# flo-audio/flo

Hardware: AMD Instinct MI355X
Metric: Msamples/s encoded (44.1k stereo, q=high) (higher is better)
Workload: dtype f32

## Files before the change

### diag/lds_model.py

```python
#!/usr/bin/env python3
import argparse
import re
from collections import Counter

import numpy as np

N, HOP, NB = 2048, 1024, 25
SLOT_CAP = 96
ROW = 1024
EDGES = np.array([0, 100, 200, 300, 400, 510, 630, 770, 920, 1080, 1270, 1480, 1720, 2000, 2320, 2700, 3150, 3700,
                  4400, 5300, 6400, 7700, 9500, 12000, 15500, 20500], dtype=np.float32)

R_WIN, R_TW, R_F1, R_F2, R_LANE, R_KEEP, R_DST, R_S10 = 0, 8, 12, 16, 20, 21, 25, 32


def bands(rate):
    res = np.float32(rate) / np.float32(N)
    band = []
    for k in range(HOP):
        f = (np.float32(k) + np.float32(0.5)) * res
        b = NB - 1
        for i in range(1, 26):
            if f < EDGES[i]:
                b = i - 1
# ... 14 lines not shown
                slot_band.append(band[k])
    dirty = 0
    for m in lane_bnd:
        dirty |= m
    band_slot0, s = [], 0
    for b in range(NB):
        band_slot0.append(s)
        while s < len(slot_band) and slot_band[s] == b:
            s += 1
    band_slot0.append(s)
    return lane_bnd, lane_slot0, band_slot0, dirty


G128 = [[0, 1, 2, 3, 12, 13, 14, 15] + list(range(20, 28)), [4, 5, 6, 7, 8, 9, 10, 11, 16, 17, 18, 19] + list(range(28, 32))]
G128 = G128 + [[l + 32 for l in g] for g in G128]
G32 = [list(range(0, 32)), list(range(32, 64))]


def contig(n):
    return [list(range(i, i + n)) for i in range(0, 64, n)]


RULES = {
    "ds_read_b32": [(G32, 1, 32)], "ds_write_b32": [(G32, 1, 32)], "ds_write_b16": [(G32, 1, 32)],
    "ds_read_b64": [(G32, 2, 64)], "ds_read_b128": [(G128, 4, 64)],
    "ds_read2_b32": [(G32, 1, 32), (G32, 1, 32)], "ds_write2_b32": [(G32, 1, 32), (G32, 1, 32)],
    "ds_read2_b64": [(contig(16), 2, 32), (contig(16), 2, 32)],
    "ds_write_b64": [(contig(16), 2, 32)], "ds_write_b128": [(contig(8), 4, 32)],
}


def cost(kind, addrs):
    acc = RULES[kind]
    lists = addrs if len(acc) == 2 else [addrs]
    cyc = base = 0
    for (groups, dw, nbank), ad in zip(acc, lists):
        for g in groups:
            per_bank = {}
            for l in g:
                if ad[l] is None:
                    continue
                for i in range(dw):
                    d = ad[l] // 4 + i
                    per_bank.setdefault(d % nbank, set()).add(d)
            cyc += max([len(v) for v in per_bank.values()] or [1])
            base += 1
    return cyc, cyc - base


def lanes(f):
    return [f(l) for l in range(64)]


def sites(rate, layout):
    lane_bnd, lane_slot0, band_slot0, dirty = band_tables(rate)
    row = lambda r, off=0: lanes(lambda l: r * ROW + 16 * l + off)
    uni = lambda a: lanes(lambda l: a)
    one = lambda a: [a] + [None] * 63
    S = []
    S += [("frame", "peek consumed / coef counters", "ds_read_b32", uni(0x8000))] * 2
    S += [("frame", "kRowS10 (uniform)", "ds_read_b128", uni(R_S10 * ROW))] * 2
    if layout == "old":
        S += [("frame", "rcount: kRowLane .z", "ds_read_b32", row(R_LANE, 8))]
    else:
        S += [("frame", "rcount: kRowS10 dword 64 + lane", "ds_read_b32", lanes(lambda l: R_S10 * ROW + 256 + 4 * l))]
    for ph, rr in (("fft pass 1", R_F1), ("fft pass 2", R_F2)):
        S += [(ph, "twiddle rows", "ds_read_b128", row(rr + k)) for k in range(3)]
        S += [(ph, "twiddle row 4 (.xy)", "ds_read_b64", row(rr + 3))]
    X = 0x10000
    for ka in range(8):
        S += [("fft exchange 1", "writes", "ds_write_b128", lanes(lambda l: X + 16 * ((8 * ka + (l & 7)) * 9 + (l >> 3))))]
    for r in range(8):
        S += [("fft exchange 1", "reads", "ds_read_b128", lanes(lambda l: X + 16 * (l * 9 + r)))]
    T = X + 16000
    S += [("masking pass", "ts_ready peek", "ds_read_b32", uni(0x8004))]
    S += [("masking pass", "ts (tl, sf)", "ds_write2_b32", [lanes(lambda l: T + 16 * (l & 31) + 4 * (l >> 5) + o if (l & 31) < 25 else None) for o in (0, 8)])]
    S += [("masking pass", "sfwh", "ds_write_b16", lanes(lambda l: T + 1024 + 2 * l if (l & 31) < 25 else None))]
    S += [("masking pass", "alive", "ds_write_b64", one(T + 1200))]
    S += [("masking pass", "ts_ready", "ds_write_b32", one(0x8004))]
    for kb in range(8):
        S += [("fft exchange 2", "writes", "ds_write_b128", lanes(lambda l: X + 16 * (((l >> 3) + 8 * kb) * 9 + (l & 7))))]
    for r in range(8):
        S += [("fft exchange 2", "reads", "ds_read_b128", lanes(lambda l: X + 16 * (l * 9 + r)))]
    pl = lambda l: 2 * l + 2 * (l >> 3)
    for r in range(8):
        if layout == "old" or r % 2 == 0:
            if layout == "old":
                S += [("post-rotation", "twiddle rows (half rows)", "ds_read_b64", row(R_TW + r // 2, 8 * (r & 1)))]
            else:
                S += [("post-rotation", "twiddle rows", "ds_read_b128", row(R_TW + r // 2))]
        S += [("post-rotation", "transpose writes (2m)", "ds_write_b64", lanes(lambda l: X + 8 * (pl(l) + 144 * r)))]
        S += [("post-rotation", "transpose writes (1023-2m)", "ds_write_b64", lanes(lambda l: X + 8 * (1149 - pl(l) - 144 * r)))]
    for q in range(8):
        S += [("post-rotation", "transpose reads", "ds_read_b128", lanes(lambda l: X + 16 * (9 * l) + 16 * q))]
    S += [("band statistics", "coef_ready", "ds_write_b32", one(0x8008))]
    es = [e for e in range(16) if (dirty >> e) & 1]
    if layout == "old":
        for rr in (R_KEEP, R_DST):
            for g in range(4):
                comp = [e - 4 * g for e in es if 4 * g <= e < 4 * g + 4 and (rr == R_DST or e < 15)]
                i = 0
                while i < len(comp):
                    if i + 1 < len(comp) and comp[i + 1] == comp[i] + 1 and comp[i] % 2 == 1:
                        S += [("band statistics", "keep / dst rows (dword pieces)", "ds_read2_b32", [row(rr + g, 4 * comp[i]), row(rr + g, 4 * comp[i] + 4)])]
                        i += 2
                    elif i + 1 < len(comp) and comp[i + 1] == comp[i] + 1:
                        S += [("band statistics", "keep / dst rows (dword pieces)", "ds_read_b64", row(rr + g, 4 * comp[i]))]
                        i += 2
                    else:
                        S += [("band statistics", "keep / dst rows (dword pieces)", "ds_read_b32", row(rr + g, 4 * comp[i]))]
                        i += 1
    else:
        S += [("band statistics", "keep / dst rows (whole rows)", "ds_read_b128", row(rr + g)) for rr in (R_KEEP, R_DST) for g in range(4)]
    SL = X + 9216
    for e in es:
        def dst(l, e=e):
            m = lane_bnd[l]
            if (m >> e) & 1:
                return SL + 16 * (lane_slot0[l] + bin(m & ((1 << e) - 1)).count("1"))
            return SL + 16 * (SLOT_CAP + l)
        S += [("band statistics", "slot stores", "ds_write_b128", lanes(dst))]
    zero = SLOT_CAP + 64
    for u in range(12):
        def src(l, u=u):
            b = min(l & 31, 24)
            bs0 = band_slot0[b] + (l >> 5)
            bs1 = band_slot0[b + 1] if (l & 31) < 25 else 0
            s = bs0 + 2 * u
            return SL + 16 * (s if s < bs1 else zero)
        S += [("band statistics", "slot gathers", "ds_read_b128", lanes(src))]
    for r in range(8):
        S += [("fold", "window rows", "ds_read_b128", row(R_WIN + r))]
    if layout == "old":
        for k in range(4):
            S += [("fold", "twiddle rows (read2_b64)", "ds_read2_b64", [row(R_TW + k), row(R_TW + k, 8)])]
    else:
        S += [("fold", "twiddle rows", "ds_read_b128", row(R_TW + k)) for k in range(4)]
    return S


def isa_mix(path):
    txt = open(path).read().split("\n")
    start = next(i for i, t in enumerate(txt) if re.match(r"^_ZN3flo20lossy_chain2q_kernelILb0ELj(\d+)ELb0EE.*:", t)
                 and "Lj65535E" not in t)
    body = txt[start:]
    e = next(i for i, t in enumerate(body) if re.match(r"^\.LBB\d+_\d+:.*_clEjS\d_S\d_S\d_S\d_\.exit", t))
    a = max(i for i, t in enumerate(body[:e]) if re.match(r"^\.LBB\d+_\d+:\s+; %\.lr\.ph\d*$", t))
    lab = body[e].split(":")[0]
    c = next(i for i, t in enumerate(body) if i > a and re.search(r"s_cbranch\w*\s+" + re.escape(lab) + r"\b", t))
    b = next(i for i, t in enumerate(body) if i > e and re.match(r"^\.LBB", t))
    mix, cold = Counter(), Counter()
    for i in range(a, b):
        m = re.search(r"\b(ds_[a-z0-9_]+)", body[i])
        if m:
            (cold if c <= i < e else mix)[m.group(1)] += 1
    return mix, cold


def main():
    ap = argparse.ArgumentParser()
    ap.add_argument("--rate", type=int, default=44100)
    ap.add_argument("--layout", default="old", choices=["old", "new"])
    ap.add_argument("--isa")
    a = ap.parse_args()
    S = sites(a.rate, a.layout)
    tab = {}
    tot_c = tot_x = 0
    for ph, site, kind, ad in S:
        c, x = cost(kind, ad)
        k = (ph, site, kind)
        n, cc, xx = tab.get(k, (0, 0, 0))
        tab[k] = (n + 1, cc + c, xx + x)
        tot_c += c
        tot_x += x
    print(f"{'phase':16} {'site':38} {'instruction':14} {'n':>3} {'array':>6} {'conflict':>8}")
    for (ph, site, kind), (n, c, x) in tab.items():
        print(f"{ph:16} {site:38} {kind:14} {n:3d} {c:6d} {x:8d}")
    print(f"{'transform wave, one stereo frame':70} {len(S):3d} {tot_c:6d} {tot_x:8d}")
    if a.isa:
        mix, cold = isa_mix(a.isa)
        model = Counter(kind for _, _, kind, _ in S)
        print("ISA mix (one frame):", dict(sorted(mix.items())), " cold loop (not run at this rate):", dict(cold))
        print("model mix          :", dict(sorted(model.items())))


if __name__ == "__main__":
    main()
```

### flo_amd/csrc/lossy_device.hpp

```cpp
#pragma once
#include <hip/hip_runtime.h>
#include <stdint.h>

#include "pack_rows.h"

namespace flo {


struct LossyDevTables {
    const float4 *pack;
    const float4 *pack_g;
    const float4 *pack_ext;
    const float *ath_db;
    const uint8_t *band;
    const float *band_count;
    const float *s10d;
    const uint32_t *lane_bnd;
    const uint32_t *lane_slot0;
    const uint32_t *band_slot0;
    int max_band_slots;
    uint32_t dirty;
    float smr_thr;
    int q_transparent;
};

constexpr int kXchStride = 9;
constexpr int kXchFloats = 64 * kXchStride * 2;
#ifdef FLO_COEF_PAD16
constexpr int kCoefFloats = 1280;
#else
constexpr int kCoefFloats = 1152;
#endif
constexpr int kSlotCap = 96;
constexpr int kFrameCap = 4352;

template <int CH>
struct WaveLds {
    union {
        float xch[CH][kXchFloats];
        float coef[CH][kCoefFloats];
        int16_t qbuf[CH][1024];
    } u;
    float2 slots[CH][kSlotCap + 64 + 1];
    float2 bandv[CH][32];
    float band_s[CH][32];
};

__device__ __forceinline__ float4 pack_row(const float4 *p) {
    typedef float v4f __attribute__((ext_vector_type(4)));
    v4f v = *reinterpret_cast<const v4f *>(p);
    asm("" : "+v"(v));
    return make_float4(v.x, v.y, v.z, v.w);
}

__device__ __forceinline__ int lane_id() { return (int)(threadIdx.x & 63); }
__device__ __forceinline__ int lane_id_opaque() {
// ... 315 lines not shown
#pragma unroll
        for (int ch = 0; ch < CH; ch++) {
            float R = fmaf(-zi[ch][r], w.y, -(zr[ch][r] * w.x));
            float I = fmaf(zi[ch][r], w.x, -(zr[ch][r] * w.y));
            coef[ch][p0] = R;
            coef[ch][p1] = I;
        }
    }
    wave_sync();
#pragma unroll
    for (int ch = 0; ch < CH; ch++) {
#ifdef FLO_COEF_PAD16
        const float4 *p = reinterpret_cast<const float4 *>(&coef[ch][20 * lane]);
#else
        const float4 *p = reinterpret_cast<const float4 *>(&coef[ch][16 * lane + 4 * (lane >> 1)]);
#endif
#pragma unroll
        for (int q = 0; q < 4; q++) {
            float4 v = p[q];
            c[ch][4 * q + 0] = v.x;
            c[ch][4 * q + 1] = v.y;
            c[ch][4 * q + 2] = v.z;
            c[ch][4 * q + 3] = v.w;
        }
    }
    wave_sync();
}

typedef float v2f __attribute__((ext_vector_type(2)));
__device__ __forceinline__ v2f fma2(v2f a, v2f b, v2f c) { return __builtin_elementwise_fma(a, b, c); }
__device__ __forceinline__ v2f fma2_na_hi_nc(v2f a, v2f w, v2f c) {
    v2f r;
    asm("v_pk_fma_f32 %0, %1, %2, %3 op_sel:[0,1,0] op_sel_hi:[1,1,1] neg_lo:[1,0,1] neg_hi:[1,0,1]" : "=v"(r) : "v"(a), "v"(w), "v"(c));
    return r;
}
__device__ __forceinline__ v2f fma2_a_hi_c(v2f a, v2f w, v2f c) {
    v2f r;
    asm("v_pk_fma_f32 %0, %1, %2, %3 op_sel:[0,1,0] op_sel_hi:[1,1,1]" : "=v"(r) : "v"(a), "v"(w), "v"(c));
    return r;
}
__device__ __forceinline__ v2f mul2_hi(v2f a, v2f w) {
    v2f r;
    asm("v_pk_mul_f32 %0, %1, %2 op_sel:[0,1] op_sel_hi:[1,1]" : "=v"(r) : "v"(a), "v"(w));
    return r;
}
__device__ __forceinline__ v2f fma2_a_hi_nc(v2f a, v2f w, v2f c) {
    v2f r;
    asm("v_pk_fma_f32 %0, %1, %2, %3 op_sel:[0,1,0] op_sel_hi:[1,1,1] neg_lo:[0,0,1] neg_hi:[0,0,1]" : "=v"(r) : "v"(a), "v"(w), "v"(c));
    return r;
}
__device__ __forceinline__ v2f splat2(float x) { return (v2f){x, x}; }

constexpr int kXch4 = 64 * kXchStride;
constexpr int kCoef2 = 1024 + 2 * 64;

__device__ __forceinline__ void dft8_2(v2f *xr, v2f *xi) {
    const v2f s = splat2(0.70710678118654752440f);
    v2f a0r = xr[0] + xr[4], a0i = xi[0] + xi[4];
    v2f a1r = xr[0] - xr[4], a1i = xi[0] - xi[4];
    v2f a2r = xr[2] + xr[6], a2i = xi[2] + xi[6];
    v2f a3r = xr[2] - xr[6], a3i = xi[2] - xi[6];
    v2f a4r = xr[1] + xr[5], a4i = xi[1] + xi[5];
    v2f a5r = xr[1] - xr[5], a5i = xi[1] - xi[5];
    v2f a6r = xr[3] + xr[7], a6i = xi[3] + xi[7];
    v2f a7r = xr[3] - xr[7], a7i = xi[3] - xi[7];
    v2f b0r = a0r + a2r, b0i = a0i + a2i;
    v2f b2r = a0r - a2r, b2i = a0i - a2i;
    v2f b1r = a1r + a3i, b1i = a1i - a3r;
    v2f b3r = a1r - a3i, b3i = a1i + a3r;
    v2f c0r = a4r + a6r, c0i = a4i + a6i;
    v2f c2r = a4r - a6r, c2i = a4i - a6i;
    v2f c1r = a5r + a7i, c1i = a5i - a7r;
    v2f c3r = a5r - a7i, c3i = a5i + a7r;
    const v2f e1r = c1r + c1i, e1i = c1i - c1r;
    const v2f e3r = c3i - c3r, e3i = c3r + c3i;
    xr[0] = b0r + c0r; xi[0] = b0i + c0i;
    xr[4] = b0r - c0r; xi[4] = b0i - c0i;
    xr[1] = fma2(e1r, s, b1r); xi[1] = fma2(e1i, s, b1i);
    xr[5] = fma2(-e1r, s, b1r); xi[5] = fma2(-e1i, s, b1i);
    xr[2] = b2r + c2i; xi[2] = b2i - c2r;
    xr[6] = b2r - c2i; xi[6] = b2i + c2r;
    xr[3] = fma2(e3r, s, b3r); xi[3] = fma2(-e3i, s, b3i);
    xr[7] = fma2(-e3r, s, b3r); xi[7] = fma2(e3i, s, b3i);
}

__device__ __forceinline__ void cmul_2(v2f &xr, v2f &xi, float wr, float wi) {
    const v2f WR = splat2(wr), WI = splat2(wi);
    v2f r = fma2(xr, WR, -(xi * WI));
    v2f i = fma2(xr, WI, xi * WR);
    xr = r;
    xi = i;
}
__device__ __forceinline__ void cmul_2_pair(v2f &xr, v2f &xi, v2f w) {
    const v2f WR = splat2(w.x);
    v2f r = fma2(xr, WR, -mul2_hi(xi, w));
    v2f i = fma2_a_hi_c(xr, w, xi * WR);
    xr = r;
    xi = i;
}

struct NoShadow { __device__ __forceinline__ void operator()() const {} };
template <typename F = NoShadow>
__device__ __forceinline__ void fft512_2(const int lane, v2f (&zr)[8], v2f (&zi)[8], float4 *x4, const LossyDevTables &T, F &&shadow = F()) {
    dft8_2(zr, zi);
#pragma unroll
    for (int kk = 0; kk < 4; kk++) {
        const float4 w = T.pack[(kRowF1 + kk) * 64 + lane];
// ... 35 lines not shown
        wave_sync();
    }
    dft8_2(zr, zi);
}

__device__ __forceinline__ void load_half_fast_2(const int lane, const float *__restrict__ pcm, long long s0, v2f (&he)[8], v2f (&ho)[8]) {
    const char *base0 = reinterpret_cast<const char *>(pcm + s0 * 2);
    const char *base1 = base0 + 4096;
    const unsigned va = 16u * (unsigned)lane, vb = 16u * (unsigned)(63 - lane);
#pragma unroll
    for (int r = 0; r < 8; r++) {
        const int rr = r & 3;
        const char *pe = (r < 4 ? base1 : base0) + va + 1024 * rr;
        const char *po = (r < 4 ? base0 : base1) + vb + (3080 - 1024 * rr);
        const float2 a = *reinterpret_cast<const float2 *>(pe);
        const float2 b = *reinterpret_cast<const float2 *>(po);
        he[r] = (v2f){a.x, a.y};
        ho[r] = (v2f){b.x, b.y};
    }
}

__device__ __forceinline__ void fold_2(const int lane, const v2f (&ae)[8], const v2f (&ao)[8], const v2f (&be)[8], const v2f (&bo)[8],
                                       v2f (&zr)[8], v2f (&zi)[8], const LossyDevTables &T) {
    float4 t4;
#pragma unroll
    for (int r = 0; r < 8; r++) {
        const float4 ww = T.pack[(kRowWin + r) * 64 + lane];
        const v2f wae = splat2(ww.x), wao = splat2(ww.y), wbe = splat2(ww.z);
        const v2f whi = {ww.z, ww.w};
        if (!(r & 1)) t4 = pack_row(&T.pack[(kRowTw + (r >> 1)) * 64 + lane]);
        const v2f wx = splat2((r & 1) ? t4.z : t4.x);
        const v2f thi = {t4.z, t4.w};
        v2f re, im;
        if (r < 4) {
            re = fma2_na_hi_nc(bo[r], whi, be[r] * wbe);
            im = fma2(ao[r], wao, -(ae[r] * wae));
        } else {
            re = fma2(-ao[r], wao, ae[r] * wae);
            im = fma2_na_hi_nc(bo[r], whi, be[r] * wbe);
        }
        if (r & 1) {
            zr[r] = fma2_na_hi_nc(im, thi, re * wx);
            zi[r] = fma2_a_hi_nc(re, thi, im * wx);
        } else {
            const v2f wy = splat2(t4.y);
            zr[r] = fma2(-im, wy, -(re * wx));
            zi[r] = fma2(re, wy, -(im * wx));
        }
    }
}

__device__ __forceinline__ void post_rotate_transpose_2(const int lane, const v2f (&zr)[8], const v2f (&zi)[8], float2 *c2,
                                                        v2f (&c)[16], const LossyDevTables &T) {
    const int pl = 2 * lane + 2 * (lane >> 3);
    float2 *const w0 = c2 + pl;
    float2 *const w1 = c2 + (1149 - 7 * 144) - pl;
    float4 t4;
#pragma unroll
    for (int r = 0; r < 8; r++) {
        if (!(r & 1)) t4 = pack_row(&T.pack[(kRowTw + (r >> 1)) * 64 + lane]);
        const v2f wx = splat2((r & 1) ? t4.z : t4.x);
        v2f R, I;
        if (r & 1) {
            const v2f thi = {t4.z, t4.w};
            R = fma2_na_hi_nc(zi[r], thi, zr[r] * wx);
            I = fma2(zi[r], wx, -mul2_hi(zr[r], thi));
        } else {
            const v2f wy = splat2(t4.y);
            R = fma2(-zi[r], wy, -(zr[r] * wx));
            I = fma2(zi[r], wx, -(zr[r] * wy));
        }
        w0[144 * r] = make_float2(R.x, R.y);
        w1[144 * (7 - r)] = make_float2(I.x, I.y);
    }
    wave_sync();
    const float4 *p = reinterpret_cast<const float4 *>(&c2[18 * lane]);
#pragma unroll
    for (int q = 0; q < 8; q++) {
        const float4 v = p[q];
        c[2 * q] = (v2f){v.x, v.y};
        c[2 * q + 1] = (v2f){v.z, v.w};
    }
    wave_sync();
}

struct LaneConst {
    float rcount;
};

__device__ __forceinline__ void load_lane_const(const int lane, LaneConst &L, const LossyDevTables &T) {
    L.rcount = T.pack[kRowLane * 64 + lane].z;
}

constexpr int kZeroSlot = kSlotCap + 64;

template <int CH>
__device__ __forceinline__ void band_stats(const int lane, const float (&c)[CH][16], float2 (*slots)[kSlotCap + 64 + 1],
                                           const LossyDevTables &T, float (&energy)[CH], float (&bmax)[CH]) {
    float kp[16];
    uint32_t dv[16], so[12];
#pragma unroll
    for (int g = 0; g < 4; g++) {
        const float4 keep = T.pack[(kRowKeep + g) * 64 + lane];
        const float4 dsto = T.pack[(kRowDst + g) * 64 + lane];
        kp[4 * g + 0] = keep.x, kp[4 * g + 1] = keep.y, kp[4 * g + 2] = keep.z, kp[4 * g + 3] = keep.w;
        dv[4 * g + 0] = __float_as_uint(dsto.x), dv[4 * g + 1] = __float_as_uint(dsto.y);
        dv[4 * g + 2] = __float_as_uint(dsto.z), dv[4 * g + 3] = __float_as_uint(dsto.w);
    }
#pragma unroll
    for (int g = 0; g < 3; g++) {
        const float4 lst = T.pack[(kRowLst + g) * 64 + lane];
        so[4 * g + 0] = __float_as_uint(lst.x), so[4 * g + 1] = __float_as_uint(lst.y);
        so[4 * g + 2] = __float_as_uint(lst.z), so[4 * g + 3] = __float_as_uint(lst.w);
    }
    __builtin_amdgcn_sched_barrier(0);
    float acc[CH], mx[CH];
#pragma unroll
    for (int ch = 0; ch < CH; ch++) {
        acc[ch] = 0.f;
        mx[ch] = 0.f;
    }
#pragma unroll
    for (int e = 0; e < 16; e++) {
#pragma unroll
        for (int ch = 0; ch < CH; ch++) {
            acc[ch] = fmaf(c[ch][e], c[ch][e], acc[ch]);
            mx[ch] = max_abs_raw(mx[ch], c[ch][e]);
            *reinterpret_cast<float2 *>(reinterpret_cast<char *>(slots[ch]) + dv[e]) = make_float2(acc[ch], mx[ch]);
            acc[ch] *= kp[e];
            mx[ch] *= kp[e];
        }
    }
    wave_sync();
    float2 v[CH][12];
// ... 929 lines not shown
```

### flo_amd/csrc/lossy_kernels.hip

```cpp
#include <assert.h>
#include <stdlib.h>

#include <mutex>
#include <set>
#include <type_traits>
#include <utility>

#include "crc_device.hpp"
#include "lossy_device.hpp"
#include "lossy_kernels.hpp"
#include "../../include/flo_synth.h"

#ifndef FLO_ABLATE
#define FLO_ABLATE 0
#endif
#ifndef FLO_SKIP
#define FLO_SKIP 0
#endif
#ifndef FLO_ABLATE3
#define FLO_ABLATE3 0
#endif
#define FLO_KEEP(x) asm volatile("" ::"v"(x))
#ifdef FLO_STAMPS
#define STAMP(i)                                                                                  \
// ... 419 lines not shown
                unsigned long long beg, len;
                crc_slice_range(total, A.parts, p, beg, len);
                const uint32_t r = crc_slice_reg<64>(tab, skip, blk_pow, byte_pow, data + beg, len, (unsigned)lane, nullptr);
                if (lane == 0) A.part_reg[(unsigned long long)clip * A.parts + p] = r;
            }
            if (lane == 0) A.crc_ready[clip] = A.epoch;
        }
        unsigned long long e = 0;
        if (lane == 0) {
            const unsigned tail = __hip_atomic_load(A.next_clip + 1, __ATOMIC_RELAXED, __HIP_MEMORY_SCOPE_AGENT);
            const unsigned head = __hip_atomic_load(A.next_clip + 2, __ATOMIC_RELAXED, __HIP_MEMORY_SCOPE_AGENT);
            if (head < tail) {
                const unsigned h = __hip_atomic_fetch_add(A.next_clip + 2, 1u, __ATOMIC_RELAXED, __HIP_MEMORY_SCOPE_AGENT);
                if (h < (unsigned)A.n_clips) e = __hip_atomic_load(A.done_q + h, __ATOMIC_RELAXED, __HIP_MEMORY_SCOPE_AGENT);
            }
        }
        const unsigned tag = (unsigned)__builtin_amdgcn_readfirstlane((int)(unsigned)(e >> 32));
        clip = (unsigned)__builtin_amdgcn_readfirstlane((int)(unsigned)e);
        if (tag != A.epoch || clip >= (unsigned)A.n_clips) return;
        __builtin_amdgcn_fence(__ATOMIC_ACQUIRE, "agent");
        asm volatile("s_waitcnt vmcnt(0)" ::: "memory");
        total = __hip_atomic_load(A.clip_bytes + clip, __ATOMIC_RELAXED, __HIP_MEMORY_SCOPE_AGENT);
    }
}

template <bool COEFFS, uint32_t DIRTY, bool DBG>
__global__ __launch_bounds__(FLO_C2X_THREADS) void lossy_chain2q_kernel(LossyArgs A, int clips_per_wg) {
    extern __shared__ __attribute__((aligned(16))) uint8_t lds_raw[];
    const int tid = (int)threadIdx.x;
    const int lane = tid & 63;
    {
        float4 *dstp = reinterpret_cast<float4 *>(lds_raw);
        for (int i = tid; i < kPackRowsHotT * 64; i += (int)blockDim.x) dstp[i] = A.T.pack[i];
        for (int i = tid; i < clips_per_wg; i += (int)blockDim.x) {
            Clip2qLds &c0 = *reinterpret_cast<Clip2qLds *>(lds_raw + kPackBytesHotT + (size_t)i * sizeof(Clip2qLds));
            c0.coef_ready = 0;
            c0.ts_ready = 0;
            c0.consumed = 0;
            c0.clip_seq = 0;
        }
        if (A.clear_next && blockIdx.x == 0 && tid == 0)
            A.clear_next[0] = A.clear_next[1] = A.clear_next[2] = 0;
    }
    __syncthreads();
    const int wv = __builtin_amdgcn_readfirstlane(tid >> 6);
    const int cl = wv % clips_per_wg;
    Clip2qLds &cs = *reinterpret_cast<Clip2qLds *>(lds_raw + kPackBytesHotT + (size_t)cl * sizeof(Clip2qLds));
    uint32_t fbase = 0, seq = 0;
    if (wv >= clips_per_wg) {
#ifndef FLO_PRIO_P
#define FLO_PRIO_P 1
#endif
        __builtin_amdgcn_s_setprio(FLO_PRIO_P);
        typedef __attribute__((address_space(3))) v4f lds_v4f;
        float athn[16];
        uint32_t ts_a[16];
        {
            const uint32_t ts0 = (uint32_t)(uintptr_t)cs.ts[0];
#pragma unroll
            for (int q = 0; q < 4; q++) {
                const float4 a4 = A.T.pack[(kRowAthN + q) * 64 + lane];
                const float4 b4 = A.T.pack[(kRowBoN + q) * 64 + lane];
                athn[4 * q + 0] = a4.x, athn[4 * q + 1] = a4.y, athn[4 * q + 2] = a4.z, athn[4 * q + 3] = a4.w;
                ts_a[4 * q + 0] = ts0 + __float_as_uint(b4.x), ts_a[4 * q + 1] = ts0 + __float_as_uint(b4.y);
                ts_a[4 * q + 2] = ts0 + __float_as_uint(b4.z), ts_a[4 * q + 3] = ts0 + __float_as_uint(b4.w);
            }
        }
        const uint32_t *const blk_g = reinterpret_cast<const uint32_t *>(A.T.pack + kRowBlk * 64);
        const uint32_t cf_a = (uint32_t)(uintptr_t)cs.u.coef2 + 16u * (uint32_t)lane + 16u * ((uint32_t)lane >> 3);
        uint8_t *const stage = cs.stage;
        const uint32_t tab_a = (uint32_t)(uintptr_t)cs.packtab;
        v4f cf[8];
        bool have = false;
        unsigned done_clip = ~0u;
        unsigned long long done_bytes = 0;
        for (;;) {
            unsigned got = 0;
            if (lane == 0) got = atomicAdd(A.next_clip, 1u);
            const unsigned clip = (unsigned)__builtin_amdgcn_readfirstlane((int)got);
            if (lane == 0) cs.clip_cur = clip;
            set_counter(&cs.clip_seq, ++seq);
            if (A.crc_ready) {
                if (clip >= (unsigned)A.n_clips) {
                    tail_crc(A, reinterpret_cast<uint32_t *>(&cs.u), lane, done_clip, done_bytes);
                    return;
                }
                if (done_clip != ~0u) tail_publish(A, done_clip, lane);
            }
            if (clip >= (unsigned)A.n_clips) return;
            const unsigned hops = A.clip_hops[clip];
            const unsigned long long frame0 = A.clip_frame0[clip];
            uint8_t *gout = A.out + A.out_off[clip];
            unsigned long long written = 0;
            uint32_t pend = 0, tailb = 0;
#ifdef FLO_STAMPS
            unsigned long long st_sum[16] = {0, 0, 0, 0, 0, 0, 0, 0, 0, 0, 0, 0, 0, 0, 0, 0}, st_last;
            asm volatile("s_memtime %0\n\ts_waitcnt lgkmcnt(0)" : "=s"(st_last)::"memory");
#endif
            for (unsigned h = 0; h < hops; h++) {
                const int ln = lane_id_opaque();
                const uint32_t g = fbase + h;
                auto take_next = [&]() __attribute__((always_inline)) {
                    if (!have && (uint32_t)__builtin_amdgcn_readfirstlane((int)peek_counter(&cs.coef_ready)) >= g + 2) {
#pragma unroll
                        for (int k = 0; k < 8; k++) cf[k] = *reinterpret_cast<const lds_v4f *>((uintptr_t)(cf_a + 1152u * (uint32_t)k));
                        set_counter(&cs.consumed, g + 2);
                        have = true;
                    }
                };
                uint32_t blk[8];
                {
                    const uint32_t *bp = blk_g;
                    asm volatile("" : "+s"(bp));
#pragma unroll
                    for (int q = 0; q < 8; q++) blk[q] = bp[q];
                }
                if (!have) {
                    wait_counter<FLO_PSLEEP>(&cs.coef_ready, g + 1);
#pragma unroll
                    for (int k = 0; k < 8; k++) cf[k] = *reinterpret_cast<const lds_v4f *>((uintptr_t)(cf_a + 1152u * (uint32_t)k));
                    set_counter(&cs.consumed, g + 1);
                }
                STAMP(0);
#ifdef FLO_STAMPS
                const unsigned long long st_frame0 = st_last;
#endif
                wait_counter<FLO_PSLEEP>(&cs.ts_ready, g + 1);
                STAMP(5);
                const uint32_t par = g & 1u;
                const uint32_t sfw_both = cs.sfwh[par][ln >> 5][ln & 31];
                const uint32_t alive = (uint32_t)__builtin_amdgcn_readfirstlane((int)(cs.alive[par][0] | cs.alive[par][1]));
                uint32_t xd[2][8];
#if (FLO_SKIP & 64) == 0
                if (par) quantise_nat<512>(cf, ts_a, athn, alive, blk, xd);
                else quantise_nat<0>(cf, ts_a, athn, alive, blk, xd);
#else
#pragma unroll
                for (int q = 0; q < 8; q++) { xd[0][q] = __float_as_uint(cf[q].x) & alive & 0x00010001u; xd[1][q] = __float_as_uint(cf[q].y) & blk[q] & 0x00010001u; }
#endif
                have = false;
                take_next();
                STAMP(1);
                if (DBG && A.dbg_q) {
#pragma unroll
                    for (int ch = 0; ch < 2; ch++) {
                        uint32_t *dq = reinterpret_cast<uint32_t *>(A.dbg_q + ((frame0 + h) * 2 + ch) * 1024);
#pragma unroll
                        for (int k = 0; k < 8; k++) dq[64 * k + ln] = xd[ch][k];
                    }
                }
                if (ln < (int)pend) stage[ln] = (uint8_t)tailb;
                uint8_t *f = stage + pend;
                const uint32_t f_a = (uint32_t)(uintptr_t)f;
                if ((ln & 31) < 25) {
                    uint8_t *p = f + 12 + 50 * (ln >> 5) + 2 * (ln & 31);
                    lds_st8<0>(p, sfw_both);
                    lds_st8<1>(p, sfw_both >> 8);
                }
                uint32_t tot[2];
                uint32_t pos = 112;
#pragma unroll
                for (int ch = 0; ch < 2; ch++) {
#if (FLO_SKIP & 32) == 0
                    uint32_t t = sparse_item_pack(ln, xd[ch], f_a + pos + 4u, tab_a);
#ifdef FLO_STAMPS
                    if (t == kSparseFallback) st_sum[6] += 1;
#endif
                    if (t == kSparseFallback) t = sparse_block_pack(ln, xd[ch], f_a + pos + 4u, tab_a);
#else
                    uint32_t t = 3u + ((xd[ch][0] | xd[ch][3]) & 1u);
                    FLO_KEEP(xd[ch][1]); FLO_KEEP(xd[ch][2]); FLO_KEEP(xd[ch][4]); FLO_KEEP(xd[ch][5]); FLO_KEEP(xd[ch][6]); FLO_KEEP(xd[ch][7]);
#endif
                    if (t == kSparseFallback) {
// ... 102 lines not shown
        asm volatile("s_memtime %0\n\ts_waitcnt lgkmcnt(0)" : "=s"(st_last)::"memory");
#endif
        v2f zr[8], zi[8];
        if (!COEFFS) fold_2(lane_id_opaque(), ae, ao, be, bo, zr, zi, T);
        float pend_e = 0.f, pend_m = 0.f;
        auto mask_publish = [&](const int ln, const uint32_t gp, const unsigned hp, const float energy1, const float bmax1,
                                const float rcount, const float4 sd0, const float4 sd1) __attribute__((always_inline)) {
            const int bnd = ln & 31, up = ln >> 5;
#if (FLO_SKIP & 16) == 0
            const float bm = bmax1;
            const float sfv1 = bm > 1e-10f ? __fdiv_rn(30000.0f, bm) : 1.0f;
            const uint32_t sfw1 = sf_word(sfv1);
            const float a = spread_threshold_2r(ln, energy1, rcount, sd0, sd1, T);
            const float sl = max_raw(a, prev * 0.7f);
            prev = sl;
            const float tl1 = masking_amplitude(sl, T.smr_thr);
#else
            const float bm = bmax1, tl1 = energy1 * 1e-3f + rcount + sd0.x + sd1.y, sfv1 = bm * 100.f + 1.f;
            const uint32_t sfw1 = __float_as_uint(tl1) >> 16;
#endif
            const unsigned long long al = __ballot(bnd < 25 && bm > tl1);
            if (bnd < 25) {
                typedef __attribute__((address_space(3))) float lds_f32;
                const uint32_t ts_s = (uint32_t)__builtin_amdgcn_readfirstlane((int)(uint32_t)(uintptr_t)cs.ts[gp & 1u]);
                lds_f32 *tp = reinterpret_cast<lds_f32 *>((uintptr_t)(ts_s + 16u * (uint32_t)bnd + 4u * (uint32_t)up));
                tp[0] = tl1;
                tp[2] = sfv1;
                cs.sfwh[gp & 1u][up][bnd] = (uint16_t)sfw1;
            }
            if (ln == 0) {
                cs.alive[gp & 1u][0] = (uint32_t)al;
                cs.alive[gp & 1u][1] = (uint32_t)(al >> 32);
            }
            if (DBG && A.dbg_sfw && bnd < 25) A.dbg_sfw[((frame0 + hp) * 2 + up) * 25 + bnd] = (unsigned short)sfw1;
            set_counter(&cs.ts_ready, gp + 1);
        };
        auto frame_body = [&](const unsigned h, v2f (&ne)[8], v2f (&no)[8], v2f (&fe)[8], v2f (&fo)[8]) __attribute__((always_inline)) {
            const int ln = lane_id_opaque();
            const uint32_t g = fbase + h;
            FLO_MARK("frame_begin");
            const uint32_t consumed_early = peek_counter(&cs.consumed);
            const float4 sd0 = T.pack[kRowS10 * 64], sd1 = T.pack[kRowS10 * 64 + 1];
            const float rcount = reinterpret_cast<const float *>(T.pack + kRowS10 * 64)[64 + ln];
            v2f c[16];
            if (COEFFS) {
#pragma unroll
                for (int q = 0; q < 4; q++) {
                    const float4 v0 = reinterpret_cast<const float4 *>(A.in_coeffs + ((frame0 + h) * 2 + 0) * 1024 + 16 * ln)[q];
                    const float4 v1 = reinterpret_cast<const float4 *>(A.in_coeffs + ((frame0 + h) * 2 + 1) * 1024 + 16 * ln)[q];
                    c[4 * q] = (v2f){v0.x, v1.x}; c[4 * q + 1] = (v2f){v0.y, v1.y};
                    c[4 * q + 2] = (v2f){v0.z, v1.z}; c[4 * q + 3] = (v2f){v0.w, v1.w};
                }
                if ((uint32_t)__builtin_amdgcn_readfirstlane((int)consumed_early) < g) wait_counter(&cs.consumed, g);
                float4 *p = reinterpret_cast<float4 *>(&cs.u.coef2[18 * ln]);
#pragma unroll
                for (int q = 0; q < 8; q++) p[q] = make_float4(c[2 * q].x, c[2 * q].y, c[2 * q + 1].x, c[2 * q + 1].y);
                wave_sync();
            } else {
                load_half_fast_2(ln, pcm, (long long)(h + 1) * 1024, ne, no);
                FLO_MARK("prefetch_done");
                STAMP(1);
                if ((uint32_t)__builtin_amdgcn_readfirstlane((int)consumed_early) < g) wait_counter(&cs.consumed, g);
                STAMP(7);
#if (FLO_SKIP & 8) == 0
                fft512_2(ln, zr, zi, cs.u.xch4, T, [&]() __attribute__((always_inline)) {
                    if (h > 0) mask_publish(ln, g - 1u, h - 1u, pend_e, pend_m, rcount, sd0, sd1);
                });
#else
                if (h > 0) mask_publish(ln, g - 1u, h - 1u, pend_e, pend_m, rcount, sd0, sd1);
#endif
                FLO_MARK("fft_done");
                STAMP(2);
#if (FLO_SKIP & 4) == 0
                post_rotate_transpose_2(ln, zr, zi, cs.u.coef2, c, T);
#else
#pragma unroll
                for (int e = 0; e < 8; e++) { c[2 * e] = zr[e]; c[2 * e + 1] = zi[e]; }
#endif
                FLO_MARK("postrot_done");
                STAMP(3);
                if (DBG && A.dbg_coeffs) {
#pragma unroll
                    for (int ch = 0; ch < 2; ch++) {
                        float *d = A.dbg_coeffs + ((frame0 + h) * 2 + ch) * 1024 + 16 * ln;
#pragma unroll
                        for (int e = 0; e < 16; e++) d[e] = ch ? c[e].y : c[e].x;
                    }
                }
            }
            set_counter(&cs.coef_ready, g + 1);
            float energy1, bmax1;
#if (FLO_SKIP & 1) == 0
            band_stats_2<DIRTY, kSoPre>(ln, c, cs.slot, T, energy1, bmax1, so_pre);
#else
            energy1 = c[0].x + c[5].y;
            bmax1 = c[1].x + c[7].y;
#endif
            FLO_MARK("bandstats_done");
            STAMP(4);
            if (COEFFS) {
                mask_publish(ln, g, h, energy1, bmax1, rcount, sd0, sd1);
            } else {
                pend_e = energy1, pend_m = bmax1;
#if (FLO_SKIP & 128) == 0
                fold_2(ln, fe, fo, ne, no, zr, zi, T);
#else
#pragma unroll
                for (int r = 0; r < 8; r++) { zr[r] = fe[r] + ne[r]; zi[r] = fo[r] - no[r]; }
#endif
// ... 985 lines not shown
```

Before: 674,000.

## Split LDS coefficient buffer into even/odd padded planes to reduce bank conflicts

Replaces the padded interleaved coefficient buffer in LDS with two even/odd planes, each padded every 64 coefficients. Post-rotation stores, the transform read-back and the packer's coefficient reads are all readdressed through a shared layout header. The goal is fewer LDS bank conflicts on the post-rotation stores and read-back. The cost is that the packer now does sixteen 64-bit reads (volatile by default) instead of eight 128-bit reads. The diagnostic model is extended to cost both layouts and to check the compiled ISA against the model.

```diff
diff --git a/diag/lds_model.py b/diag/lds_model.py
--- a/diag/lds_model.py
+++ b/diag/lds_model.py
@@ -90,7 +90,64 @@
     return [f(l) for l in range(64)]
 
 
-def sites(rate, layout):
+class CoefPadded:
+    elems = 1024 + 2 * 64
+
+    @staticmethod
+    def elem(k):
+        return k + 2 * (k >> 4)
+
+    @classmethod
+    def readback(cls, l):
+        return [("ds_read_b128", 8 * cls.elem(16 * l + 2 * q), (2 * q, 2 * q + 1)) for q in range(8)]
+
+    @classmethod
+    def packer(cls, l):
+        return [("ds_read_b128", 8 * cls.elem(128 * b + 2 * l), (128 * b + 2 * l, 128 * b + 2 * l + 1)) for b in range(8)]
+
+
+class CoefPlanes:
+    plane = 512 + 2 * 16
+    elems = 2 * plane
+
+    @classmethod
+    def elem(cls, k):
+        return (k & 1) * cls.plane + (k >> 1) + 2 * (k >> 6)
+
+    @classmethod
+    def readback(cls, l):
+        return [("ds_read_b128", 8 * cls.elem(16 * l + 4 * t + p), (4 * t + p, 4 * t + p + 2)) for p in range(2) for t in range(4)]
+
+    @classmethod
+    def packer(cls, l):
+        return [("ds_read_b64", 8 * cls.elem(128 * b + 2 * l + h), (128 * b + 2 * l + h,)) for b in range(8) for h in range(2)]
+
+
+COEF_LAYOUTS = {"padded": CoefPadded, "planes": CoefPlanes}
+
+
+def coef_patterns(coef, base=0x10000):
+    L = COEF_LAYOUTS[coef]
+    st = []
+    for r in range(8):
+        st += [("ds_write_b64", lanes(lambda l: base + 8 * L.elem(2 * (l + 64 * r))))]
+        st += [("ds_write_b64", lanes(lambda l: base + 8 * L.elem(1023 - 2 * (l + 64 * r))))]
+    rb = [(L.readback(0)[i][0], lanes(lambda l: base + L.readback(l)[i][1])) for i in range(len(L.readback(0)))]
+    pk = [(L.packer(0)[i][0], lanes(lambda l: base + L.packer(l)[i][1])) for i in range(len(L.packer(0)))]
+    return {"post-rotation stores": st, "transform read-back": rb, "packer reads": pk}
+
+
+def coef_costs(coef):
+    out = {}
+    for name, acc in coef_patterns(coef).items():
+        cs = [cost(kind, ad) for kind, ad in acc]
+        out[name] = (len(acc), sum(c for c, _ in cs), sum(x for _, x in cs))
+    return out
+
+
+
+
+def sites(rate, layout, coef="planes"):
     lane_bnd, lane_slot0, band_slot0, dirty = band_tables(rate)
     row = lambda r, off=0: lanes(lambda l: r * ROW + 16 * l + off)
     uni = lambda a: lanes(lambda l: a)
@@ -120,17 +177,16 @@
         S += [("fft exchange 2", "writes", "ds_write_b128", lanes(lambda l: X + 16 * (((l >> 3) + 8 * kb) * 9 + (l & 7))))]
     for r in range(8):
         S += [("fft exchange 2", "reads", "ds_read_b128", lanes(lambda l: X + 16 * (l * 9 + r)))]
-    pl = lambda l: 2 * l + 2 * (l >> 3)
+    cp = coef_patterns(coef, X)
     for r in range(8):
         if layout == "old" or r % 2 == 0:
             if layout == "old":
                 S += [("post-rotation", "twiddle rows (half rows)", "ds_read_b64", row(R_TW + r // 2, 8 * (r & 1)))]
             else:
                 S += [("post-rotation", "twiddle rows", "ds_read_b128", row(R_TW + r // 2))]
-        S += [("post-rotation", "transpose writes (2m)", "ds_write_b64", lanes(lambda l: X + 8 * (pl(l) + 144 * r)))]
-        S += [("post-rotation", "transpose writes (1023-2m)", "ds_write_b64", lanes(lambda l: X + 8 * (1149 - pl(l) - 144 * r)))]
-    for q in range(8):
-        S += [("post-rotation", "transpose reads", "ds_read_b128", lanes(lambda l: X + 16 * (9 * l) + 16 * q))]
+        S += [("post-rotation", "transpose writes (2m)", *cp["post-rotation stores"][2 * r])]
+        S += [("post-rotation", "transpose writes (1023-2m)", *cp["post-rotation stores"][2 * r + 1])]
+    S += [("post-rotation", "transpose reads", kind, ad) for kind, ad in cp["transform read-back"]]
     S += [("band statistics", "coef_ready", "ds_write_b32", one(0x8008))]
     es = [e for e in range(16) if (dirty >> e) & 1]
     if layout == "old":
@@ -181,27 +237,57 @@
     txt = open(path).read().split("\n")
     start = next(i for i, t in enumerate(txt) if re.match(r"^_ZN3flo20lossy_chain2q_kernelILb0ELj(\d+)ELb0EE.*:", t)
                  and "Lj65535E" not in t)
-    body = txt[start:]
-    e = next(i for i, t in enumerate(body) if re.match(r"^\.LBB\d+_\d+:.*_clEjS\d_S\d_S\d_S\d_\.exit", t))
-    a = max(i for i, t in enumerate(body[:e]) if re.match(r"^\.LBB\d+_\d+:\s+; %\.lr\.ph\d*$", t))
-    lab = body[e].split(":")[0]
-    c = next(i for i, t in enumerate(body) if i > a and re.search(r"s_cbranch\w*\s+" + re.escape(lab) + r"\b", t))
-    b = next(i for i, t in enumerate(body) if i > e and re.match(r"^\.LBB", t))
+    end = next(i for i in range(start, len(txt)) if "s_endpgm" in txt[i])
+    body = txt[start:end]
+    heads = [i for i, t in enumerate(body) if re.match(r"^\.LBB\d+_\d+:", t) and any("This Loop Header: Depth=2" in u for u in body[i:i + 2])]
+
+    def loop(h):
+        name = body[h].split(":")[0][2:]
+        last = max(i for i, t in enumerate(body) if re.search(r"(Header=|Parent Loop )" + name + r"\b", t))
+        e = next((i for i in range(last + 1, len(body)) if re.match(r"^\.LBB\d+_\d+:", body[i])), len(body))
+        return body[h:e]
+
+    frame = loop(heads[-1])
+    label_at = {t.split(":")[0]: i for i, t in enumerate(frame) if re.match(r"^\.LBB\d+_\d+:", t)}
+    targets = {}
+    for i, t in enumerate(frame):
+        m = re.search(r"s_cbranch\w*\s+(\.LBB\d+_\d+)\b", t)
+        if m and label_at.get(m.group(1), -1) > i:
+            targets.setdefault(m.group(1), []).append(i)
+    spans = [(v[0], label_at[k]) for k, v in targets.items() if len(v) >= 3]
     mix, cold = Counter(), Counter()
-    for i in range(a, b):
-        m = re.search(r"\b(ds_[a-z0-9_]+)", body[i])
+    for i, t in enumerate(frame):
+        m = re.match(r"^\s+(ds_[a-z0-9_]+)", t)
         if m:
-            (cold if c <= i < e else mix)[m.group(1)] += 1
-    return mix, cold
+            (cold if any(a <= i < b for a, b in spans) else mix)[m.group(1)] += 1
+    packer, run, takes = Counter(), Counter(), 0
+    for t in loop(heads[0]) + [""]:
+        m = re.match(r"^\s+(ds_read_b64|ds_read_b128|ds_read2_b64)\b", t)
+        if m:
+            run[m.group(1)] += 1
+        elif not re.match(r"^\s+(s_waitcnt|s_nop|;)", t):
+            if sum(run.values()) >= 8:
+                packer += run
+                takes += 1
+            run = Counter()
+    half = lambda c, n=2: {k: v // n for k, v in c.items() if v % n == 0 or not print("uneven", k, v)}
+    return Counter(half(mix)), Counter(half(cold)), Counter(half(packer, max(takes, 1)))
+
+
+def isa_accepts(mix, cold, packer, S, coef):
+    model = Counter(kind for _, _, kind, _ in S)
+    want = Counter(kind for kind, _ in coef_patterns(coef)["packer reads"])
+    return dict(mix) == dict(model) and set(cold) <= {"ds_read_b128"} and dict(packer) == dict(want)
 
 
 def main():
     ap = argparse.ArgumentParser()
     ap.add_argument("--rate", type=int, default=44100)
     ap.add_argument("--layout", default="old", choices=["old", "new"])
+    ap.add_argument("--coef-layout", default="planes", choices=sorted(COEF_LAYOUTS))
     ap.add_argument("--isa")
     a = ap.parse_args()
-    S = sites(a.rate, a.layout)
+    S = sites(a.rate, a.layout, a.coef_layout)
     tab = {}
     tot_c = tot_x = 0
     for ph, site, kind, ad in S:
@@ -215,11 +301,18 @@
     for (ph, site, kind), (n, c, x) in tab.items():
         print(f"{ph:16} {site:38} {kind:14} {n:3d} {c:6d} {x:8d}")
     print(f"{'transform wave, one stereo frame':70} {len(S):3d} {tot_c:6d} {tot_x:8d}")
+    print(f"coefficient buffer, layout '{a.coef_layout}' ({COEF_LAYOUTS[a.coef_layout].elems} elements):")
+    for name, (n, c, x) in coef_costs(a.coef_layout).items():
+        print(f"{'':16} {name:53} {n:3d} {c:6d} {x:8d}")
     if a.isa:
-        mix, cold = isa_mix(a.isa)
+        mix, cold, packer = isa_mix(a.isa)
         model = Counter(kind for _, _, kind, _ in S)
         print("ISA mix (one frame):", dict(sorted(mix.items())), " cold loop (not run at this rate):", dict(cold))
         print("model mix          :", dict(sorted(model.items())))
+        print("packer, one take   :", dict(sorted(packer.items())))
+        ok = isa_accepts(mix, cold, packer, S, a.coef_layout)
+        print("listing matches the model" if ok else "listing DIFFERS from the model")
+        raise SystemExit(0 if ok else 1)
 
 
 if __name__ == "__main__":
diff --git a/flo_amd/csrc/coef_layout.h b/flo_amd/csrc/coef_layout.h
--- /dev/null
+++ b/flo_amd/csrc/coef_layout.h
@@ -0,0 +1,37 @@
+#pragma once
+#include <cstdint>
+
+namespace flo {
+namespace coef_layout {
+constexpr uint32_t kElemBytes = 8;
+constexpr uint32_t kPlaneElems = 512 + 2 * 16;
+constexpr uint32_t kElems = 2 * kPlaneElems;
+constexpr uint32_t kBytes = kElems * kElemBytes;
+constexpr uint32_t kPlaneBytes = kPlaneElems * kElemBytes;
+
+constexpr uint32_t elem(uint32_t k) { return (k & 1u) * kPlaneElems + (k >> 1) + 2u * (k >> 6); }
+constexpr uint32_t byte_of(uint32_t k) { return kElemBytes * elem(k); }
+
+constexpr uint32_t store_lane_byte(uint32_t lane) { return 8u * lane + 16u * (lane >> 5); }
+constexpr uint32_t kStoreRowBytes = 68 * kElemBytes;
+constexpr uint32_t kStoreIBase = (kElems - 3) * kElemBytes;
+constexpr uint32_t store_r_byte(uint32_t lane, uint32_t r) { return store_lane_byte(lane) + kStoreRowBytes * r; }
+constexpr uint32_t store_i_byte(uint32_t lane, uint32_t r) { return kStoreIBase - store_lane_byte(lane) - kStoreRowBytes * r; }
+constexpr uint32_t store_r_coef(uint32_t lane, uint32_t r) { return 2u * (lane + 64u * r); }
+constexpr uint32_t store_i_coef(uint32_t lane, uint32_t r) { return 1023u - 2u * (lane + 64u * r); }
+
+constexpr uint32_t read_lane_byte(uint32_t lane) { return 64u * lane + 16u * (lane >> 2); }
+constexpr uint32_t read_off_byte(uint32_t q) { return (q >> 2) * kPlaneBytes + 16u * (q & 3u); }
+constexpr uint32_t read_byte(uint32_t lane, uint32_t q) { return read_lane_byte(lane) + read_off_byte(q); }
+constexpr uint32_t read_coef_lo(uint32_t q) { return 4u * (q & 3u) + (q >> 2); }
+constexpr uint32_t read_coef_hi(uint32_t q) { return read_coef_lo(q) + 2u; }
+
+constexpr uint32_t pack_lane_byte(uint32_t lane) { return 8u * lane + 16u * (lane >> 5); }
+constexpr uint32_t pack_off_byte(uint32_t b, uint32_t h) { return h * kPlaneBytes + kStoreRowBytes * b; }
+constexpr uint32_t pack_byte(uint32_t lane, uint32_t b, uint32_t h) { return pack_lane_byte(lane) + pack_off_byte(b, h); }
+constexpr uint32_t pack_coef(uint32_t lane, uint32_t b, uint32_t h) { return 128u * b + 2u * lane + h; }
+
+static_assert(elem(1023) * kElemBytes == kStoreIBase, "the I stores count down from coefficient 1023");
+static_assert(elem(1022) + 1 == kPlaneElems - 2 && elem(1023) + 3 == kElems, "each plane ends in its last padding pair");
+}
+}
diff --git a/flo_amd/csrc/lossy_device.hpp b/flo_amd/csrc/lossy_device.hpp
--- a/flo_amd/csrc/lossy_device.hpp
+++ b/flo_amd/csrc/lossy_device.hpp
@@ -2,6 +2,7 @@
 #include <hip/hip_runtime.h>
 #include <stdint.h>
 
+#include "coef_layout.h"
 #include "pack_rows.h"
 
 namespace flo {
@@ -423,7 +424,8 @@
 __device__ __forceinline__ v2f splat2(float x) { return (v2f){x, x}; }
 
 constexpr int kXch4 = 64 * kXchStride;
-constexpr int kCoef2 = 1024 + 2 * 64;
+constexpr int kCoef2 = (int)coef_layout::kElems;
+static_assert(kCoef2 * 8 <= kXch4 * 16, "the coefficient buffer fits the FFT exchange it shares its memory with");
 
 __device__ __forceinline__ void dft8_2(v2f *xr, v2f *xi) {
     const v2f s = splat2(0.70710678118654752440f);
@@ -565,9 +567,9 @@
 
 __device__ __forceinline__ void post_rotate_transpose_2(const int lane, const v2f (&zr)[8], const v2f (&zi)[8], float2 *c2,
                                                         v2f (&c)[16], const LossyDevTables &T) {
-    const int pl = 2 * lane + 2 * (lane >> 3);
-    float2 *const w0 = c2 + pl;
-    float2 *const w1 = c2 + (1149 - 7 * 144) - pl;
+    namespace cl = coef_layout;
+    char *const w0 = reinterpret_cast<char *>(c2) + cl::store_lane_byte((uint32_t)lane);
+    char *const w1 = reinterpret_cast<char *>(c2) + (cl::kStoreIBase - 7 * cl::kStoreRowBytes) - cl::store_lane_byte((uint32_t)lane);
     float4 t4;
 #pragma unroll
     for (int r = 0; r < 8; r++) {
@@ -583,16 +585,16 @@
             R = fma2(-zi[r], wy, -(zr[r] * wx));
             I = fma2(zi[r], wx, -(zr[r] * wy));
         }
-        w0[144 * r] = make_float2(R.x, R.y);
-        w1[144 * (7 - r)] = make_float2(I.x, I.y);
+        *reinterpret_cast<float2 *>(w0 + (int)cl::kStoreRowBytes * r) = make_float2(R.x, R.y);
+        *reinterpret_cast<float2 *>(w1 + (int)cl::kStoreRowBytes * (7 - r)) = make_float2(I.x, I.y);
     }
     wave_sync();
-    const float4 *p = reinterpret_cast<const float4 *>(&c2[18 * lane]);
+    const char *p = reinterpret_cast<const char *>(c2) + cl::read_lane_byte((uint32_t)lane);
 #pragma unroll
     for (int q = 0; q < 8; q++) {
-        const float4 v = p[q];
-        c[2 * q] = (v2f){v.x, v.y};
-        c[2 * q + 1] = (v2f){v.z, v.w};
+        const float4 v = *reinterpret_cast<const float4 *>(p + cl::read_off_byte((uint32_t)q));
+        c[cl::read_coef_lo((uint32_t)q)] = (v2f){v.x, v.y};
+        c[cl::read_coef_hi((uint32_t)q)] = (v2f){v.z, v.w};
     }
     wave_sync();
 }
diff --git a/flo_amd/csrc/lossy_kernels.hip b/flo_amd/csrc/lossy_kernels.hip
--- a/flo_amd/csrc/lossy_kernels.hip
+++ b/flo_amd/csrc/lossy_kernels.hip
@@ -495,7 +495,6 @@
 #define FLO_PRIO_P 1
 #endif
         __builtin_amdgcn_s_setprio(FLO_PRIO_P);
-        typedef __attribute__((address_space(3))) v4f lds_v4f;
         float athn[16];
         uint32_t ts_a[16];
         {
@@ -510,10 +509,23 @@
             }
         }
         const uint32_t *const blk_g = reinterpret_cast<const uint32_t *>(A.T.pack + kRowBlk * 64);
-        const uint32_t cf_a = (uint32_t)(uintptr_t)cs.u.coef2 + 16u * (uint32_t)lane + 16u * ((uint32_t)lane >> 3);
+        const uint32_t cf_a = (uint32_t)(uintptr_t)cs.u.coef2 + coef_layout::pack_lane_byte((uint32_t)lane);
         uint8_t *const stage = cs.stage;
         const uint32_t tab_a = (uint32_t)(uintptr_t)cs.packtab;
         v4f cf[8];
+#ifdef FLO_CF_READ2
+        typedef __attribute__((address_space(3))) v2f lds_v2f;
+#else
+        typedef volatile __attribute__((address_space(3))) v2f lds_v2f;
+#endif
+        auto take_coefs = [&]() __attribute__((always_inline)) {
+#pragma unroll
+            for (int k = 0; k < 8; k++) {
+                const v2f e = *reinterpret_cast<const lds_v2f *>((uintptr_t)(cf_a + coef_layout::pack_off_byte((uint32_t)k, 0)));
+                const v2f o = *reinterpret_cast<const lds_v2f *>((uintptr_t)(cf_a + coef_layout::pack_off_byte((uint32_t)k, 1)));
+                cf[k] = (v4f){e.x, e.y, o.x, o.y};
+            }
+        };
         bool have = false;
         unsigned done_clip = ~0u;
         unsigned long long done_bytes = 0;
@@ -545,8 +557,7 @@
                 const uint32_t g = fbase + h;
                 auto take_next = [&]() __attribute__((always_inline)) {
                     if (!have && (uint32_t)__builtin_amdgcn_readfirstlane((int)peek_counter(&cs.coef_ready)) >= g + 2) {
-#pragma unroll
-                        for (int k = 0; k < 8; k++) cf[k] = *reinterpret_cast<const lds_v4f *>((uintptr_t)(cf_a + 1152u * (uint32_t)k));
+                        take_coefs();
                         set_counter(&cs.consumed, g + 2);
                         have = true;
                     }
@@ -560,8 +571,7 @@
                 }
                 if (!have) {
                     wait_counter<FLO_PSLEEP>(&cs.coef_ready, g + 1);
-#pragma unroll
-                    for (int k = 0; k < 8; k++) cf[k] = *reinterpret_cast<const lds_v4f *>((uintptr_t)(cf_a + 1152u * (uint32_t)k));
+                    take_coefs();
                     set_counter(&cs.consumed, g + 1);
                 }
                 STAMP(0);
@@ -770,9 +780,12 @@
                     c[4 * q + 2] = (v2f){v0.z, v1.z}; c[4 * q + 3] = (v2f){v0.w, v1.w};
                 }
                 if ((uint32_t)__builtin_amdgcn_readfirstlane((int)consumed_early) < g) wait_counter(&cs.consumed, g);
-                float4 *p = reinterpret_cast<float4 *>(&cs.u.coef2[18 * ln]);
-#pragma unroll
-                for (int q = 0; q < 8; q++) p[q] = make_float4(c[2 * q].x, c[2 * q].y, c[2 * q + 1].x, c[2 * q + 1].y);
+                char *p = reinterpret_cast<char *>(cs.u.coef2) + coef_layout::read_lane_byte((uint32_t)ln);
+#pragma unroll
+                for (int q = 0; q < 8; q++) {
+                    const v2f lo = c[coef_layout::read_coef_lo((uint32_t)q)], hi = c[coef_layout::read_coef_hi((uint32_t)q)];
+                    *reinterpret_cast<float4 *>(p + coef_layout::read_off_byte((uint32_t)q)) = make_float4(lo.x, lo.y, hi.x, hi.y);
+                }
                 wave_sync();
             } else {
                 load_half_fast_2(ln, pcm, (long long)(h + 1) * 1024, ne, no);
```

Result: no change. 678,900 (median of 6 runs) (+0.7%).
